# COMP6248-Reproducability-Challenge/selfsupervised-denoising

Measured on AMD Instinct MI355X. Metric: training patches/sec (64x64 gauss25 SSDN), higher is better.
Workload: dtype f16

## Files before the change

include/ssdn_hip.h:

```cpp
#ifndef SSDN_HIP_H
#define SSDN_HIP_H

#include <stdint.h>

#ifdef __cplusplus
extern "C" {
#endif
#if defined(__GNUC__) || defined(__clang__)
#pragma GCC visibility push(default)
#endif

#define SSDN_ABI_VERSION 19
#define SSDN_MAX_TAPS 9

typedef struct ssdn_view {
    void* p;
    int32_t cs;
    int32_t co;
} ssdn_view;

enum ssdn_op_type {
    SSDN_OP_PACK_INPUT = 1,
    SSDN_OP_CONV = 2,
    SSDN_OP_POOL_FWD = 3,
// ... 427 lines not shown
    const float* w_e;
    const float* w_d;
    float* out;
    int32_t B, C, H, W;
    int32_t R;
    int32_t ntaps;
    int32_t dy[SSDN_MAX_TAPS], dx[SSDN_MAX_TAPS];
    const float* add;
} ssdn_input_grad_args;

int ssdn_run_ops(const ssdn_op* ops, int n, void* stream);

int ssdn_stream_order(void* first, void* then);

int ssdn_conv_lds_bytes(const ssdn_conv_args* a);
int ssdn_wgrad_lds_bytes(const ssdn_wgrad_args* a);
int ssdn_wgrad_mega_ok(const ssdn_wgrad_args* a);
int ssdn_wgrad_variant(const ssdn_wgrad_args* a, int32_t* out9);
int ssdn_conv_dma_split(const ssdn_conv_args* a, int32_t* out8);

int ssdn_struct_size(int op_type);
int ssdn_abi_version(void);
const char* ssdn_last_error(void);
int ssdn_device_cus(void);

#define SSDN_PROF_CONV_MT3 0
#define SSDN_PROF_CONV_MT2 1
#define SSDN_PROF_CONV_MT1 2
#define SSDN_PROF_WGRAD 3
#define SSDN_PROF_GEMM 4
#define SSDN_PROF_CDMA_MT3 5
#define SSDN_PROF_CDMA_MT21 6
#define SSDN_PROF_WGRAD_SIDE 7
#define SSDN_PROF_KINDS 8
int ssdn_profile_enable(int kind, int max_launches);
int ssdn_profile_set_stride(int kind, int stride);
int ssdn_profile_read(int kind, double* total_ms, long long* launches, double* flops, double* bytes);

int ssdn_conv_set_mode(int mode);
int ssdn_conv_fuses_pool(const ssdn_conv_args* a);
int ssdn_conv_fuses_upsum(const ssdn_conv_args* a);
int ssdn_conv_fuses_unrot(const ssdn_conv_args* a);
int ssdn_conv_fuses_urot(const ssdn_conv_args* a);
int ssdn_conv_signs(const ssdn_conv_args* a);
int ssdn_conv16_eligible(const ssdn_conv_args* a);
int ssdn_conv_set_conv16(int roles);

int ssdn_chain_len(const ssdn_op* ops, int n);
int ssdn_conv_set_chain(int on);

int ssdn_wgrad_mergeable(const ssdn_wgrad_args* a);

#define SSDN_PLAN_REPACK 0
#define SSDN_PLAN_FORWARD 1
#define SSDN_PLAN_BACKWARD 2
#define SSDN_PLAN_OPTIMISER 3
#define SSDN_PLAN_PHASES 4
typedef struct ssdn_plan ssdn_plan;
int ssdn_plan_load(const void* blob, int64_t nbytes, ssdn_plan** out);
void ssdn_plan_destroy(ssdn_plan* plan);
int64_t ssdn_plan_arena_bytes(const ssdn_plan* plan);
const char* ssdn_plan_meta(const ssdn_plan* plan);
int ssdn_plan_bind(ssdn_plan* plan, void* arena);
int ssdn_plan_tensor(const ssdn_plan* plan, const char* name, void** ptr, int64_t* bytes);
int ssdn_plan_run(ssdn_plan* plan, int phase, void* stream);
int ssdn_plan_set_lr(ssdn_plan* plan, float lr, int step, float gscale);
int ssdn_net_forward(ssdn_plan* plan, void* stream);
int ssdn_train_step(ssdn_plan* plan, float lr, int step, void* stream);

void ssdn_debug_set_trace(void* device_buffer);
void* ssdn_debug_get_trace(void);

int ssdn_probe_mfma(const void* a_frag, const void* b_frag, float* d_out, void* stream);
int ssdn_probe_tr16(const void* lds_image, int image_bytes, const int32_t* lane_addr, void* out, void* stream);

#if defined(__GNUC__) || defined(__clang__)
#pragma GCC visibility pop
#endif
#ifdef __cplusplus
}
#endif
#endif
// ... 1 lines not shown
```

selfsupervised-denoising_amd/csrc/api.hip:

```cpp
#include "common.h"
#include <cstdarg>
#include <cstdio>
#include <cstdlib>

static thread_local char g_err[512] = "";
thread_local hipEvent_t g_ssdn_stop_event = nullptr;
thread_local bool g_ssdn_stop_used = false;
thread_local hipEvent_t g_ssdn_prof_start = nullptr, g_ssdn_prof_stop = nullptr;
thread_local bool g_ssdn_prof_used = false;

int ssdn_set_error(const char* fmt, ...) {
    va_list ap;
    va_start(ap, fmt);
    vsnprintf(g_err, sizeof(g_err), fmt, ap);
    va_end(ap);
    return -1;
}

#include <vector>
struct ProfSlot {
    bool on = false;
    std::vector<hipEvent_t> ev;
    size_t used = 0;
    double flops = 0.0, bytes = 0.0;
// ... 137 lines not shown
int ssdn_conv_lds_bytes(const ssdn_conv_args* a) { return conv_lds_bytes(a); }
int ssdn_wgrad_lds_bytes(const ssdn_wgrad_args* a) { return wgrad_lds_bytes(a); }
int ssdn_wgrad_mergeable(const ssdn_wgrad_args* a) { return a && wgrad_mergeable(a) ? 1 : 0; }
int ssdn_wgrad_mega_ok(const ssdn_wgrad_args* a) { return wgrad_mega_ok(a); }
int ssdn_conv_fuses_pool(const ssdn_conv_args* a) { return a && conv_fuses_pool(a) ? 1 : 0; }
int ssdn_conv_fuses_upsum(const ssdn_conv_args* a) { return a && conv_fuses_upsum(a) ? 1 : 0; }
int ssdn_conv_fuses_unrot(const ssdn_conv_args* a) { return a && conv_fuses_unrot(a) ? 1 : 0; }
int ssdn_conv_fuses_urot(const ssdn_conv_args* a) { return a && conv_fuses_urot(a) ? 1 : 0; }
int ssdn_conv_signs(const ssdn_conv_args* a) { return a && conv_signs(a) ? 1 : 0; }
int ssdn_conv16_eligible(const ssdn_conv_args* a) { return a && conv_use_conv16(a) ? 1 : 0; }

#define SSDN_NEVENTS 256
#define SSDN_NLANES 4
#define SSDN_MAX_DEVICES 16
struct LaneSet {
    hipStream_t side[SSDN_NLANES] = {nullptr, nullptr, nullptr, nullptr};
    hipEvent_t ev[SSDN_NEVENTS];
    int ev_next = 0;
    bool ready = false;
};
static LaneSet g_lanesets[SSDN_MAX_DEVICES];
static LaneSet* lanes_get() {
    int dev = 0;
    if (hipGetDevice(&dev) != hipSuccess || dev < 0 || dev >= SSDN_MAX_DEVICES) { ssdn_set_error("lanes: bad current device"); return nullptr; }
    LaneSet& L = g_lanesets[dev];
    if (L.ready) return &L;
    for (int l = 1; l < SSDN_NLANES; ++l)
        if (hipStreamCreateWithFlags(&L.side[l], hipStreamNonBlocking) != hipSuccess) { ssdn_set_error("lanes: hipStreamCreate failed"); return nullptr; }
    for (int i = 0; i < SSDN_NEVENTS; ++i)
        if (hipEventCreateWithFlags(&L.ev[i], hipEventDisableTiming) != hipSuccess) { ssdn_set_error("lanes: hipEventCreate failed"); return nullptr; }
    L.ready = true;
    return &L;
}
static const unsigned g_lane_deps[SSDN_NLANES] = {0u, 1u << 0, (1u << 0) | (1u << 1) | (1u << 3), 1u << 0};

int ssdn_stream_order(void* first, void* then) {
    LaneSet* LS = lanes_get();
    if (!LS) return -1;
    hipEvent_t e = LS->ev[LS->ev_next++ % SSDN_NEVENTS];
    SSDN_CHECK_HIP(hipEventRecord(e, (hipStream_t)first));
    SSDN_CHECK_HIP(hipStreamWaitEvent((hipStream_t)then, e, 0));
    return 0;
}

int ssdn_run_ops(const ssdn_op* ops, int n, void* stream) {
    hipStream_t lane_s[SSDN_NLANES] = {(hipStream_t)stream, nullptr, nullptr, nullptr};
    g_ssdn_stop_event = nullptr;
    bool dirty[SSDN_NLANES][SSDN_NLANES] = {}, used[SSDN_NLANES] = {true, false, false, false};
    for (int d = 1; d < SSDN_NLANES; ++d) dirty[0][d] = true;
    static const bool one_lane = ssdn_tuning_env("SSDN_ONE_LANE") != nullptr;
    LaneSet* LS = nullptr;
    hipEvent_t cover[SSDN_NLANES] = {nullptr, nullptr, nullptr, nullptr};
    bool covered[SSDN_NLANES] = {false, false, false, false};
    long long cover_at[SSDN_NLANES] = {0, 0, 0, 0};
    auto cover_live = [&](int l) { return covered[l] && (!LS || (long long)LS->ev_next - cover_at[l] < SSDN_NEVENTS - 1); };
    bool has_side = false;
    static const bool no_stop = ssdn_tuning_env("SSDN_NO_STOP_EVENTS") != nullptr;
    for (int i = 0; i < n && !one_lane; ++i) has_side = has_side || ops[i].lane > 0;
    if (has_side && !(LS = lanes_get())) return -1;
    for (int i = 0; i < n; ++i) {
        const void* p = ops[i].args;
        int rc = 0;
        if (!p) return ssdn_set_error("op %d: null args", i);
        int lane = one_lane ? 0 : ops[i].lane;
        if (lane < 0 || lane >= SSDN_NLANES) return ssdn_set_error("op %d: bad lane %d", i, lane);
        if (lane > 0) {
// ... 106 lines not shown
                        if (ok < 0) return -1;
                        if (ok) {
                            arm_last(ia + 1 + mp);
                            rc = launch_tail_fused(items, m, ad, packs, mp, s);
                            i = ia + mp;
                            break;
                        }
                    }
                }
                arm_last(i + m);
                rc = m > 1 ? launch_wreduce_multi(items, m, s) : launch_wreduce((const ssdn_wreduce_args*)p, s);
                i += m - 1;
                break;
            }
            case SSDN_OP_WPACK: {
                const ssdn_wpack_args* items[WPACK_MULTI_MAX];
                int m = 0;
                while (m < WPACK_MULTI_MAX && i + m < n && ops[i + m].type == SSDN_OP_WPACK && ops[i + m].args &&
                       (one_lane ? 0 : ops[i + m].lane) == lane)
                    items[m] = (const ssdn_wpack_args*)ops[i + m].args, ++m;
                rc = m > 1 ? launch_wpack_multi(items, m, s) : launch_wpack((const ssdn_wpack_args*)p, s);
                i += m - 1;
                break;
            }
            case SSDN_OP_GRAD_PACK: {
                const bool next_conv = i + 1 < n && ops[i + 1].type == SSDN_OP_CONV && ops[i + 1].args && (one_lane ? 0 : ops[i + 1].lane) == lane;
                if (next_conv && chain_merging_on() && conv_gradpack_fusable((const ssdn_grad_pack_args*)p, (const ssdn_conv_args*)ops[i + 1].args)) {
                    arm(i + 2);
                    rc = launch_gradpack_dgrad((const ssdn_grad_pack_args*)p, (const ssdn_conv_args*)ops[i + 1].args, s);
                    ++i;
                } else { arm(i + 1); rc = launch_grad_pack((const ssdn_grad_pack_args*)p, s); }
                break;
            }
            case SSDN_OP_HEAD_SSDN: rc = launch_head((const ssdn_head_args*)p, s); break;
            case SSDN_OP_HEAD_FINAL: rc = launch_head_final((const ssdn_head_final_args*)p, s); break;
            case SSDN_OP_SPATIAL_MEAN: rc = launch_spatial_mean((const ssdn_spatial_mean_args*)p, s); break;
            case SSDN_OP_MSE: rc = launch_mse((const ssdn_mse_args*)p, 0, s); break;
            case SSDN_OP_MASK_MSE: rc = launch_mse((const ssdn_mse_args*)p, 1, s); break;
            case SSDN_OP_ADAM: {
                const ssdn_wpack_args* items[ADAM_PACK_MAX];
                int m = 0;
                while (m < ADAM_PACK_MAX && i + 1 + m < n && ops[i + 1 + m].type == SSDN_OP_WPACK && ops[i + 1 + m].args &&
                       (one_lane ? 0 : ops[i + 1 + m].lane) == lane)
                    items[m] = (const ssdn_wpack_args*)ops[i + 1 + m].args, ++m;
                const bool whole_run = !(i + 1 + m < n && ops[i + 1 + m].type == SSDN_OP_WPACK);
                if (m > 0 && whole_run && adam_pack_fusable((const ssdn_adam_args*)p, items, m)) {
                    rc = launch_adam_pack((const ssdn_adam_args*)p, items, m, s);
                    i += m;
                } else rc = launch_adam((const ssdn_adam_args*)p, s);
                break;
            }
            case SSDN_OP_METRICS: rc = launch_metrics((const ssdn_metrics_args*)p, s); break;
            case SSDN_OP_NOISE: rc = launch_noise((const ssdn_noise_args*)p, s); break;
            case SSDN_OP_INPUT_GRAD: arm(i + 1); rc = launch_input_grad((const ssdn_input_grad_args*)p, s); break;
            case SSDN_OP_HEAD_VJP: rc = launch_head_vjp((const ssdn_head_vjp_args*)p, s); break;
            case SSDN_OP_MSE_VJP: rc = launch_mse_vjp((const ssdn_mse_vjp_args*)p, s); break;
            case SSDN_OP_ACCUM: rc = launch_accum((const ssdn_accum_args*)p, s); break;
            case SSDN_OP_HEAD_POSTERIOR: rc = launch_head_posterior((const ssdn_head_posterior_args*)p, s); break;
            case SSDN_OP_SSIM: rc = launch_ssim((const ssdn_ssim_args*)p, s); break;
            case SSDN_OP_CALIBRATION: rc = launch_calibration((const ssdn_calibration_args*)p, s); break;
            case SSDN_OP_IMAGE_IN: rc = launch_image_in((const ssdn_image_in_args*)p, s); break;
            case SSDN_OP_IMAGE_OUT: rc = launch_image_out((const ssdn_image_out_args*)p, s); break;
            case SSDN_OP_NOISE_EST: rc = launch_noise_est((const ssdn_noise_est_args*)p, s); break;
            case SSDN_OP_TILE_IN: rc = launch_tile_in((const ssdn_tile_in_args*)p, s); break;
            case SSDN_OP_TILE_OUT: rc = launch_tile_out((const ssdn_tile_out_args*)p, s); break;
            case SSDN_OP_POOL_PATCH: rc = launch_pool_patch((const ssdn_pool_patch_args*)p, s); break;
            case SSDN_OP_ZERO: {
// ... 75 lines not shown
```

selfsupervised-denoising_amd/csrc/common.h:

```cpp
#pragma once
#include <hip/hip_runtime.h>
#include <hip/hip_ext.h>
#include <stdint.h>
#include "../../include/ssdn_hip.h"
#include <cstdlib>

#if defined(SSDN_TUNING)
static inline const char* ssdn_tuning_env(const char* name) { return std::getenv(name); }
#else
static inline const char* ssdn_tuning_env(const char*) { return nullptr; }
#endif

typedef _Float16 h16;
typedef _Float16 half8 __attribute__((ext_vector_type(8)));
typedef _Float16 half4 __attribute__((ext_vector_type(4)));
typedef _Float16 half2v __attribute__((ext_vector_type(2)));
typedef __bf16 bf16x8 __attribute__((ext_vector_type(8)));
typedef unsigned short u16x8 __attribute__((ext_vector_type(8)));
typedef unsigned short u16x4 __attribute__((ext_vector_type(4)));
typedef float f32x16 __attribute__((ext_vector_type(16)));
typedef float f32x4 __attribute__((ext_vector_type(4)));

#define LRELU_SLOPE 0.1f

// ... 72 lines not shown
static inline int ssdn_current_device_slot() {
    int dev = 0;
    if (hipGetDevice(&dev) != hipSuccess || dev < 0) dev = 0;
    return dev % SSDN_MAX_DEVICES_ATTR;
}

void prof_begin(int kind, hipStream_t s);
void prof_end(int kind, hipStream_t s, double flops, double bytes);

int launch_conv(const ssdn_conv_args* a, hipStream_t s);
int launch_wgrad(const ssdn_wgrad_args* a, hipStream_t s);
bool wgrad_mergeable(const ssdn_wgrad_args* a);
int launch_wgrad_multi(const ssdn_wgrad_args* const* items, int n, hipStream_t s);
#define WGRAD_MEGA_MAX 64
int wgrad_mega_ok(const ssdn_wgrad_args* a);
int launch_wgrad_mega(const ssdn_wgrad_args* const* ops, int n, hipStream_t s);
int launch_pack_input(const ssdn_pack_input_args* a, hipStream_t s);
int launch_pool_fwd(const ssdn_pool_args* a, hipStream_t s);
int launch_pool_bwd(const ssdn_pool_args* a, hipStream_t s);
int launch_upsum_bwd(const ssdn_upsum_args* a, hipStream_t s);
int launch_unrot_fwd(const ssdn_unrot_args* a, hipStream_t s);
int launch_unrot_bwd(const ssdn_unrot_args* a, hipStream_t s);
int launch_wreduce(const ssdn_wreduce_args* a, hipStream_t s);
int launch_wpack(const ssdn_wpack_args* a, hipStream_t s);
#define WPACK_MULTI_MAX 24
int launch_wpack_multi(const ssdn_wpack_args* const* items, int n, hipStream_t s);
#define WREDUCE_MULTI_MAX 32
#define WGRAD_MULTI_MAX 32
int launch_wreduce_multi(const ssdn_wreduce_args* const* items, int n, hipStream_t s);
int launch_grad_pack(const ssdn_grad_pack_args* a, hipStream_t s);
int launch_head(const ssdn_head_args* a, hipStream_t s);
int launch_head_impulse(const ssdn_head_args* a, hipStream_t s);
int launch_head_final(const ssdn_head_final_args* a, hipStream_t s);
int launch_spatial_mean(const ssdn_spatial_mean_args* a, hipStream_t s);
int launch_mse(const ssdn_mse_args* a, int masked, hipStream_t s);
int launch_head_vjp(const ssdn_head_vjp_args* a, hipStream_t s);
int launch_head_vjp_impulse(const ssdn_head_vjp_args* a, hipStream_t s);
int launch_head_posterior(const ssdn_head_posterior_args* a, hipStream_t s);
int launch_ssim(const ssdn_ssim_args* a, hipStream_t s);
int launch_calibration(const ssdn_calibration_args* a, hipStream_t s);
int launch_image_in(const ssdn_image_in_args* a, hipStream_t s);
int launch_image_out(const ssdn_image_out_args* a, hipStream_t s);
int launch_noise_est(const ssdn_noise_est_args* a, hipStream_t s);
int launch_tile_in(const ssdn_tile_in_args* a, hipStream_t s);
int launch_tile_out(const ssdn_tile_out_args* a, hipStream_t s);
int launch_pool_patch(const ssdn_pool_patch_args* a, hipStream_t s);
int launch_mse_vjp(const ssdn_mse_vjp_args* a, hipStream_t s);
int launch_adam(const ssdn_adam_args* a, hipStream_t s);
#define ADAM_PACK_MAX 24
int adam_pack_fusable(const ssdn_adam_args* a, const ssdn_wpack_args* const* items, int n);
int launch_adam_pack(const ssdn_adam_args* a, const ssdn_wpack_args* const* items, int n, hipStream_t s);
int tail_fused_ok(const ssdn_wreduce_args* const* wr, int nw, const ssdn_adam_args* a, const ssdn_wpack_args* const* wp, int np);
int launch_tail_fused(const ssdn_wreduce_args* const* wr, int nw, const ssdn_adam_args* a, const ssdn_wpack_args* const* wp, int np, hipStream_t s);
int launch_metrics(const ssdn_metrics_args* a, hipStream_t s);
int launch_accum(const ssdn_accum_args* a, hipStream_t s);
int launch_noise(const ssdn_noise_args* a, hipStream_t s);
int launch_input_grad(const ssdn_input_grad_args* a, hipStream_t s);
int conv_lds_bytes(const ssdn_conv_args* a);
int conv_validate(const ssdn_conv_args* a);
int chain_len(const ssdn_op* ops, int n, bool any_lane);
int launch_chain(const ssdn_op* ops, int n, bool any_lane, hipStream_t s);
bool chain_merging_on();
bool conv_dma_eligible(const ssdn_conv_args* a, bool any_size);
int conv_dma_lds_bytes(int mt);
bool conv_signs(const ssdn_conv_args* a);
bool gemm_dma_signs(const ssdn_conv_args* a);
// ... 32 lines not shown
```

selfsupervised-denoising_amd/csrc/head.hip:

```cpp
#include "head_math.h"

static constexpr float PME_EPS = 1e-6f;
static __device__ __forceinline__ float diag_pme_weights(float sx, float sn, float& ix, float& in, float& u, float& v) {
    const float e = PME_EPS;
    ix = 1.f / (sx + e);
    in = 1.f / (sn + e);
    const float rD = 1.f / (ix + in + e);
    u = ix * rD;
    v = in * rD;
    return rD;
}

static __device__ __forceinline__ float gauss3_pme_adj(const Sym3& s, Sym3& k) {
    return 1.f / sym3_adj(sym3_add_diag(s, 2 * PME_EPS, 2 * PME_EPS, 2 * PME_EPS), k);
}
template <bool DIAG>
__global__ void k_head(ssdn_head_args a) {
    __shared__ float sh[4];
    const int b = blockIdx.y;
    const long long HW = (long long)a.H * a.W;
    const int C = a.C;
    const int Cout = DIAG ? 2 * C : C + C * (C + 1) / 2;
    const float inv_total = 1.f / ((float)a.B * (float)HW);
    const HeadEst he = head_est(a.mode, a.est_raw, b);
    const float est = he.est, dest_draw = he.dest_draw;
    const float npar = a.noise_param ? a.noise_param[b] : 0.f;
    float loss_acc = 0.f, gest_acc = 0.f, gabs = 0.f;
    const HeadRange r = head_range(HW, a.nchunks);
    const long long p0 = r.p0, p1 = r.p1;
    const float* no = a.net_out + (long long)b * Cout * HW;
    const float* ny = a.noisy + (long long)b * C * HW;
    for (long long p = p0 + threadIdx.x; p < p1; p += HB) {
        if constexpr (DIAG) {
            float mu[3], av[3], sig[3], dsig_dmu[3], dsig_dest[3], sx[3], sn[3], rs[3], q[3];
            float prod = 1.f, quad = 0.f;
#pragma unroll
            for (int c = 0; c < 3; ++c) {
                mu[c] = no[c * HW + p];
                av[c] = no[(3 + c) * HW + p];
                head_sigma(a.style, a.mode, npar, est, mu[c], sig[c], dsig_dmu[c], dsig_dest[c]);
                sx[c] = av[c] * av[c];
                sn[c] = sig[c] * sig[c];
                const float sy = sx[c] + sn[c], d = ny[c * HW + p] - mu[c];
                rs[c] = 1.f / sy;
                q[c] = d * rs[c];
                prod *= sy;
                quad += d * q[c];
            }
            float l = 0.5f * logf(fmaxf(prod, 0.f)) + 0.5f * quad;
            if (a.mode != 0) l -= 0.1f * (sig[0] + sig[1] + sig[2]) * (1.f / 3.f);
            loss_acc += l;
            long long o3 = (long long)b * 3 * HW + p;
            if (a.mu) { a.mu[o3] = mu[0]; a.mu[o3 + HW] = mu[1]; a.mu[o3 + 2 * HW] = mu[2]; }
            if (a.pme) {
#pragma unroll
                for (int c = 0; c < 3; ++c) {
                    float ix, in, u, v;
                    diag_pme_weights(sx[c], sn[c], ix, in, u, v);
                    a.pme[o3 + c * HW] = mu[c] * u + ny[c * HW + p] * v;
                }
            }
            if (a.model_std) a.model_std[(long long)b * HW + p] = cbrtf(fabsf(av[0] * av[1] * av[2]));
            if (a.noise_std && a.style == 1) a.noise_std[(long long)b * HW + p] = cbrtf(sig[0] * sig[1] * sig[2]);
            if (a.want_grad) {
                const float hd = prod > 0.f ? 0.5f : 0.f;
// ... 68 lines not shown
                float t00 = s00 + 2 * e, t11 = s11 + 2 * e, t22 = s22 + 2 * e;
                float k00 = t11 * t22 - s12 * s12, k01 = s02 * s12 - s01 * t22, k02 = s01 * s12 - s02 * t11;
                float k11 = t00 * t22 - s02 * s02, k12 = s01 * s02 - t00 * s12, k22 = t00 * t11 - s01 * s01;
                float rd = 1.f / (t00 * k00 + s01 * k01 + s02 * k02);
                float r0 = (k00 * d0 + k01 * d1 + k02 * d2) * rd;
                float r1 = (k01 * d0 + k11 * d1 + k12 * d2) * rd;
                float r2 = (k02 * d0 + k12 * d1 + k22 * d2) * rd;
                a.pme[o3] = mu[0] + (x00 + e) * r0 + x01 * r1 + x02 * r2;
                a.pme[o3 + HW] = mu[1] + x01 * r0 + (x11 + e) * r1 + x12 * r2;
                a.pme[o3 + 2 * HW] = mu[2] + x02 * r0 + x12 * r1 + (x22 + e) * r2;
            }
            if (a.model_std) a.model_std[(long long)b * HW + p] = cbrtf(fabsf(A[0] * A[3] * A[5]));
            if (a.noise_std && a.style == 1) a.noise_std[(long long)b * HW + p] = cbrtf(sig[0] * sig[1] * sig[2]);
            if (a.want_grad) {
                float hd = det > 0.f ? 0.5f : 0.f;
                const Sym3 G = {hd * i00 - 0.5f * q0 * q0, hd * i01 - 0.5f * q0 * q1, hd * i02 - 0.5f * q0 * q2,
                                hd * i11 - 0.5f * q1 * q1, hd * i12 - 0.5f * q1 * q2, hd * i22 - 0.5f * q2 * q2};
                float reg = a.mode != 0 ? 0.1f / 3.f : 0.f;
                float ds0 = 2.f * sig[0] * G.m00 - reg, ds1 = 2.f * sig[1] * G.m11 - reg, ds2 = 2.f * sig[2] * G.m22 - reg;
                float g[9];
                g[0] = -q0 + ds0 * dsig_dmu[0];
                g[1] = -q1 + ds1 * dsig_dmu[1];
                g[2] = -q2 + ds2 * dsig_dmu[2];
                sym3_dldu(G, A, g + 3);
#pragma unroll
                for (int c = 0; c < 9; ++c) {
                    float v = g[c] * inv_total;
                    a.g_net_out[((long long)b * 9 + c) * HW + p] = v;
                    gabs = fmaxf(gabs, fabsf(v));
                }
                gest_acc += ds0 * dsig_dest[0] + ds1 * dsig_dest[1] + ds2 * dsig_dest[2];
            }
        }
    }
    float ls = block_sum(loss_acc, sh);
    float gs = block_sum(gest_acc, sh);
    if (threadIdx.x == 0) {
        float* pp = a.partial + ((long long)b * a.nchunks + blockIdx.x) * 2;
        pp[0] = ls;
        pp[1] = gs * dest_draw * inv_total;
    }
    if (a.want_grad && a.gmax) atomic_max_abs_block(a.gmax, gabs, sh);
    if (blockIdx.x == 0 && threadIdx.x == 0 && a.noise_std && a.style == 0)
        a.noise_std[b] = head_sigma(0, a.mode, npar, est, 0.f);
}
template <class Args>
static int check_head_args(const char* op, const Args* a, bool need_g) {
    if (a->diag && a->C != 1 && a->C != 3) return ssdn_set_error("%s: diag needs C = 1 or 3", op);
    if (a->C != 1 && a->C != 3) return ssdn_set_error("%s: C must be 1 or 3 (denoiser.py:199)", op);
    if (a->diag != 0 && a->diag != 1) return ssdn_set_error("%s: diag must be 0 or 1", op);
    if (a->B < 1 || a->H < 1 || a->W < 1 || a->nchunks < 1) return ssdn_set_error("%s: bad shape", op);
    if (a->mode < 0 || a->mode > 2 || a->style < 0 || a->style > 2) return ssdn_set_error("%s: bad style / mode", op);
    if (!a->net_out || !a->noisy || !a->partial) return ssdn_set_error("%s: net_out, noisy and partial must be given", op);
    if (need_g && !a->g_net_out) return ssdn_set_error("%s: g_net_out must be given", op);
    if (a->mode == 0 && !a->noise_param) return ssdn_set_error("%s: mode known needs noise_param", op);
    if (a->mode != 0 && !a->est_raw) return ssdn_set_error("%s: modes const / var need est_raw", op);
    return 0;
}
int launch_head(const ssdn_head_args* a, hipStream_t s) {
    if (int rc = check_head_args("head", a, a->want_grad != 0)) return rc;
    if (a->style == 2) return launch_head_impulse(a, s);
    if (a->diag && a->C == 3) hipLaunchKernelGGL(k_head<true>, dim3(a->nchunks, a->B), dim3(HB), 0, s, *a);
    else hipLaunchKernelGGL(k_head<false>, dim3(a->nchunks, a->B), dim3(HB), 0, s, *a);
    return 0;
}

__global__ void k_head_final(ssdn_head_final_args a) {
    int b = blockIdx.x * blockDim.x + threadIdx.x;
    long long HW = (long long)a.H * a.W;
    if (b < a.B) {
        float l = 0.f, g = 0.f;
        for (int c = 0; c < a.nchunks; ++c) {
            l += a.partial[((long long)b * a.nchunks + c) * 2];
            g += a.partial[((long long)b * a.nchunks + c) * 2 + 1];
        }
        if (a.loss) a.loss[b] = l / (float)HW;
        if (a.mode == 2 && a.g_est) a.g_est[b] = g;
    }
    if (a.mode == 1 && a.g_est && b == 0) {
        float g = 0.f;
        for (int bb = 0; bb < a.B; ++bb)
            for (int c = 0; c < a.nchunks; ++c) g += a.partial[((long long)bb * a.nchunks + c) * 2 + 1];
        a.g_est[0] = g;
    }
}
__global__ void k_fill_sigma_grad(ssdn_head_final_args a) {
    long long idx = (long long)blockIdx.x * blockDim.x + threadIdx.x;
    long long HW = (long long)a.H * a.W;
    if (idx >= a.B * HW) return;
    int b = idx / HW;
    float v = a.g_est[b] / (float)HW;
    a.g_sigma_out[idx] = v;
    if ((idx % HW) == 0 && v != 0.f && a.gmax2) atomicMax(a.gmax2, __float_as_uint(fabsf(v)));
}
int launch_head_final(const ssdn_head_final_args* a, hipStream_t s) {
    hipLaunchKernelGGL(k_head_final, dim3((a->B + 63) / 64), dim3(64), 0, s, *a);
    if (a->mode == 2 && a->g_sigma_out) {
        long long n = (long long)a->B * a->H * a->W;
        hipLaunchKernelGGL(k_fill_sigma_grad, dim3((int)((n + 255) / 256)), dim3(256), 0, s, *a);
    }
    return 0;
}

__global__ void k_spatial_mean(ssdn_spatial_mean_args a) {
    __shared__ float sh[4];
    int b = blockIdx.x;
    float acc = 0.f;
    for (int i = threadIdx.x; i < a.HW; i += HB) acc += a.src[(long long)b * a.HW + i];
    float t = block_sum(acc, sh);
    if (threadIdx.x == 0) a.dst[b] = t / (float)a.HW;
}
int launch_spatial_mean(const ssdn_spatial_mean_args* a, hipStream_t s) {
    hipLaunchKernelGGL(k_spatial_mean, dim3(a->B), dim3(HB), 0, s, *a);
    return 0;
}

__global__ void k_mse(ssdn_mse_args a) {
    __shared__ float sh[4];
    int b = blockIdx.x;
    long long n = (long long)a.C * a.H * a.W;
    float acc = 0.f, gabs = 0.f;
    float k = 2.f / ((float)n * (float)a.B);
    for (long long i = threadIdx.x; i < n; i += HB) {
        float d = a.out[b * n + i] - a.ref[b * n + i];
        acc += d * d;
        if (a.g) {
            float g = k * d;
            a.g[b * n + i] = g;
            gabs = fmaxf(gabs, fabsf(g));
        }
    }
    float t = block_sum(acc, sh);
    if (threadIdx.x == 0) a.loss[b] = t / (float)n;
// ... 471 lines not shown
```

selfsupervised-denoising_amd/csrc/head_common.h:

```cpp
#pragma once
#include "common.h"

#define HB 256

static __device__ __forceinline__ float block_sum(float v, float* sh) {
#pragma unroll
    for (int o = 32; o > 0; o >>= 1) v += __shfl_down(v, o, 64);
    int w = threadIdx.x >> 6, l = threadIdx.x & 63;
    __syncthreads();
    if (l == 0) sh[w] = v;
    __syncthreads();
    return sh[0] + sh[1] + sh[2] + sh[3];
}
static __device__ __forceinline__ void atomic_max_abs(uint32_t* gmax, float v) {
    float a = fabsf(v);
#pragma unroll
    for (int o = 32; o > 0; o >>= 1) a = fmaxf(a, __shfl_down(a, o, 64));
    if ((threadIdx.x & 63) == 0 && a > 0.f) atomicMax(gmax, __float_as_uint(a));
}
static __device__ __forceinline__ void atomic_max_abs_block(uint32_t* gmax, float v, float* sh4) {
    float a = fabsf(v);
#pragma unroll
    for (int o = 32; o > 0; o >>= 1) a = fmaxf(a, __shfl_down(a, o, 64));
    __syncthreads();
    if ((threadIdx.x & 63) == 0) sh4[threadIdx.x >> 6] = a;
    __syncthreads();
    if (threadIdx.x == 0) {
        const float m = fmaxf(fmaxf(sh4[0], sh4[1]), fmaxf(sh4[2], sh4[3]));
        if (m > 0.f) atomicMax(gmax, __float_as_uint(m));
    }
}
static __device__ __forceinline__ float softplus_m4(float raw) {
    float x = raw - 4.f;
    return (x > 20.f ? x : log1pf(expf(x))) + 1e-3f;
}
static __device__ __forceinline__ float sigmoid_m4(float raw) {
    float x = raw - 4.f;
    return x > 20.f ? 1.f : 1.f / (1.f + expf(-x));
}
```

selfsupervised-denoising_amd/ssdn/hip/lib.py:

```python
from __future__ import annotations

import ctypes as C
import os

_HERE = os.path.dirname(os.path.abspath(__file__))
LIB_PATH = os.environ.get("SSDN_HIP_LIB") or os.path.join(_HERE, "libssdn_hip.so")
MAX_TAPS = 9

OP = dict(pack_input=1, conv=2, pool_fwd=3, pool_bwd=4, upsum_bwd=5, unrot_fwd=6, unrot_bwd=7, wgrad=8, wreduce=9,
          wpack=10, grad_pack=11, head_ssdn=12, head_final=13, spatial_mean=14, mse=15, mask_mse=16, adam=17,
          metrics=18, zero=19, event_record=20, noise=21, input_grad=22, head_vjp=23,
          mse_vjp=24, accum=25, head_posterior=26, ssim=27, calibration=28, image_in=29, image_out=30, noise_est=31,
          tile_in=32, tile_out=33, pool_patch=34)

i32, f32, vp = C.c_int32, C.c_float, C.c_void_p


class View(C.Structure):
    _fields_ = [("p", vp), ("cs", i32), ("co", i32)]


class OpRec(C.Structure):
    _fields_ = [("type", i32), ("lane", i32), ("args", vp)]

# ... 168 lines not shown
                ("k0", i32), ("B", i32), ("dst", vp)]


class TileOutArgs(C.Structure):
    _fields_ = [("store", vp), ("w", i32), ("h", i32), ("C", i32), ("T", i32), ("O", i32), ("Kx", i32), ("Ky", i32), ("mode", i32),
                ("dst", vp), ("dst_bytes", C.c_int64)]


class PoolPatchArgs(C.Structure):
    _fields_ = [("pool", vp), ("offsets", vp), ("sizes", vp), ("params", vp), ("index", vp), ("noisy32", vp), ("ref32", vp), ("coords", vp),
                ("param_out", vp), ("origin_out", vp), ("N", i32), ("B", i32), ("C", i32), ("P", i32), ("augment", i32),
                ("n2v_box", i32), ("n2v_radius", i32), ("seed", C.c_uint64), ("offset", C.c_uint64)]


def tile_count(n: int, T: int, O: int) -> int:
    return 1 if n <= T else -(-(n - O) // (T - O))


ARG_TYPES = dict(pack_input=PackInputArgs, conv=ConvArgs, pool_fwd=PoolArgs, pool_bwd=PoolArgs, upsum_bwd=UpsumArgs,
                 unrot_fwd=UnrotArgs, unrot_bwd=UnrotArgs, wgrad=WgradArgs, wreduce=WreduceArgs, wpack=WpackArgs,
                 grad_pack=GradPackArgs, head_ssdn=HeadArgs, head_final=HeadFinalArgs, spatial_mean=SpatialMeanArgs,
                 mse=MseArgs, mask_mse=MseArgs, adam=AdamArgs, metrics=MetricsArgs, zero=ZeroArgs, event_record=EventArgs, noise=NoiseArgs,
                 input_grad=InputGradArgs, head_vjp=HeadVjpArgs, mse_vjp=MseVjpArgs, accum=AccumArgs,
                 head_posterior=HeadPosteriorArgs, ssim=SsimArgs, calibration=CalibrationArgs, image_in=ImageInArgs, image_out=ImageOutArgs,
                 noise_est=NoiseEstArgs, tile_in=TileInArgs, tile_out=TileOutArgs, pool_patch=PoolPatchArgs)

ABI_VERSION = 19

SYMBOLS = ["ssdn_run_ops", "ssdn_stream_order", "ssdn_conv_lds_bytes", "ssdn_wgrad_lds_bytes", "ssdn_abi_version", "ssdn_last_error",
           "ssdn_device_cus", "ssdn_probe_mfma", "ssdn_probe_tr16", "ssdn_struct_size", "ssdn_profile_enable",
           "ssdn_profile_read", "ssdn_profile_set_stride", "ssdn_debug_set_trace", "ssdn_debug_get_trace", "ssdn_conv_set_mode",
           "ssdn_wgrad_mergeable", "ssdn_conv_fuses_pool", "ssdn_conv_fuses_upsum", "ssdn_conv_fuses_unrot", "ssdn_conv_fuses_urot", "ssdn_conv_signs", "ssdn_chain_len",
           "ssdn_conv_set_chain", "ssdn_wgrad_mega_ok", "ssdn_wgrad_variant", "ssdn_conv_dma_split", "ssdn_conv16_eligible", "ssdn_conv_set_conv16",
           "ssdn_plan_load", "ssdn_plan_destroy", "ssdn_plan_arena_bytes", "ssdn_plan_meta", "ssdn_plan_bind", "ssdn_plan_tensor", "ssdn_plan_run",
           "ssdn_plan_set_lr", "ssdn_net_forward", "ssdn_train_step"]
PLAN_PHASES = dict(repack=0, forward=1, backward=2, optimiser=3)
PROF = dict(conv_mt3=0, conv_mt2=1, conv_mt1=2, wgrad=3, gemm=4, cdma_mt3=5, cdma_mt21=6, wgrad_side=7)

CONV_SIGN_FIELDS = ("unrot_smask", "urot_smask", "sign_out", "mask_sign", "upsum_mask_sign")


def conv_args(a: dict, view, ptr) -> ConvArgs:
    s = ConvArgs()
    s.src0, s.src1 = view(a["src0"]), view(a["src1"])
    s.c0, s.c1, s.up0, s.N, s.H, s.W, s.ntaps = a["c0"], a["c1"], a["up0"], a["N"], a["H"], a["W"], len(a["taps"])
    for t, (dy, dx) in enumerate(a["taps"]):
        s.dy[t], s.dx[t] = dy, dx
    s.w, s.wc = ptr("w", a["layer"]), ptr("wc", a["layer"])
    s.M, s.Mpad, s.Ktot, s.act = a["M"], a["Mpad"], a["Ktot"], a["act"]
    s.bias = ptr("bias", a["layer"]) if a["bias"] else None
    s.mask, s.add, s.dst = view(a["mask"]), view(a["add"]), view(a["dst"])
    s.dst32 = ptr("dst32", a["dst32"]) if a["dst32"] is not None else None
    s.ltw, s.lth, s.ltn, s.kc, s.bf16, s.kreal = a["ltw"], a["lth"], a["ltn"], a["kc"], a["bf16"], a.get("kreal", 0)
    s.pool, s.pool_shifted = view(a.get("pool")), a.get("pool_shifted", 0)
    s.upsum, s.upsum_mask, s.upsum_c = view(a.get("upsum")), view(a.get("upsum_mask")), a.get("upsum_c", 0)
    s.unrot, s.unrot_mask, s.urot = view(a.get("unrot")), view(a.get("unrot_mask")), view(a.get("urot"))
    for k in CONV_SIGN_FIELDS:
        setattr(s, k, ptr(k, a[k]) if a.get(k) is not None else None)
    return s


def pointer_fields(st, base: int = 0):
    out = []
    for name, ty in st._fields_:
        off = base + getattr(st, name).offset
        if ty is vp:
            out.append(off)
        elif isinstance(ty, type) and issubclass(ty, C.Structure):
            out += pointer_fields(ty, off)
    return out
# ... 27 lines not shown
    lib.ssdn_last_error.restype = C.c_char_p
    lib.ssdn_device_cus.restype = C.c_int
    lib.ssdn_probe_mfma.argtypes = [vp, vp, vp, vp]
    lib.ssdn_probe_mfma.restype = C.c_int
    lib.ssdn_probe_tr16.argtypes = [vp, C.c_int, vp, vp, vp]
    lib.ssdn_probe_tr16.restype = C.c_int
    lib.ssdn_profile_enable.argtypes = [C.c_int, C.c_int]
    lib.ssdn_profile_enable.restype = C.c_int
    lib.ssdn_profile_set_stride.argtypes = [C.c_int, C.c_int]
    lib.ssdn_profile_set_stride.restype = C.c_int
    lib.ssdn_profile_read.argtypes = [C.c_int, C.POINTER(C.c_double), C.POINTER(C.c_longlong), C.POINTER(C.c_double), C.POINTER(C.c_double)]
    lib.ssdn_profile_read.restype = C.c_int
    lib.ssdn_conv_set_mode.argtypes = [C.c_int]
    lib.ssdn_conv_set_mode.restype = C.c_int
    lib.ssdn_conv_set_chain.argtypes = [C.c_int]
    lib.ssdn_conv_set_chain.restype = C.c_int
    lib.ssdn_chain_len.argtypes = [C.c_void_p, C.c_int]
    lib.ssdn_chain_len.restype = C.c_int
    lib.ssdn_conv_fuses_unrot.argtypes = [C.c_void_p]
    lib.ssdn_conv_fuses_unrot.restype = C.c_int
    lib.ssdn_conv_fuses_urot.argtypes = [C.c_void_p]
    lib.ssdn_conv_fuses_urot.restype = C.c_int
    lib.ssdn_conv_signs.argtypes = [C.c_void_p]
    lib.ssdn_conv_signs.restype = C.c_int
    lib.ssdn_conv_fuses_upsum.argtypes = [C.c_void_p]
    lib.ssdn_conv_fuses_upsum.restype = C.c_int
    lib.ssdn_conv_fuses_pool.argtypes = [C.c_void_p]
    lib.ssdn_conv_fuses_pool.restype = C.c_int
    if hasattr(lib, "ssdn_conv16_eligible"):
        lib.ssdn_conv16_eligible.argtypes = [C.c_void_p]
        lib.ssdn_conv16_eligible.restype = C.c_int
        lib.ssdn_conv_set_conv16.argtypes = [C.c_int]
        lib.ssdn_conv_set_conv16.restype = C.c_int
    lib.ssdn_wgrad_mergeable.argtypes = [C.c_void_p]
    lib.ssdn_wgrad_mergeable.restype = C.c_int
    lib.ssdn_wgrad_mega_ok.argtypes = [C.c_void_p]
    lib.ssdn_wgrad_mega_ok.restype = C.c_int
    lib.ssdn_wgrad_variant.argtypes = [C.c_void_p, C.POINTER(C.c_int32)]
    lib.ssdn_wgrad_variant.restype = C.c_int
    if hasattr(lib, "ssdn_conv_dma_split"):
        lib.ssdn_conv_dma_split.argtypes = [C.c_void_p, C.POINTER(C.c_int32)]
        lib.ssdn_conv_dma_split.restype = C.c_int
    lib.ssdn_struct_size.argtypes = [C.c_int]
    lib.ssdn_struct_size.restype = C.c_int
    lib.ssdn_plan_load.argtypes = [C.c_void_p, C.c_int64, C.POINTER(C.c_void_p)]
    lib.ssdn_plan_load.restype = C.c_int
    lib.ssdn_plan_destroy.argtypes = [C.c_void_p]
    lib.ssdn_plan_destroy.restype = None
    lib.ssdn_plan_arena_bytes.argtypes = [C.c_void_p]
    lib.ssdn_plan_arena_bytes.restype = C.c_int64
    lib.ssdn_plan_meta.argtypes = [C.c_void_p]
    lib.ssdn_plan_meta.restype = C.c_char_p
    lib.ssdn_plan_bind.argtypes = [C.c_void_p, C.c_void_p]
    lib.ssdn_plan_bind.restype = C.c_int
    lib.ssdn_plan_tensor.argtypes = [C.c_void_p, C.c_char_p, C.POINTER(C.c_void_p), C.POINTER(C.c_int64)]
    lib.ssdn_plan_tensor.restype = C.c_int
    lib.ssdn_plan_run.argtypes = [C.c_void_p, C.c_int, C.c_void_p]
    lib.ssdn_plan_run.restype = C.c_int
    lib.ssdn_plan_set_lr.argtypes = [C.c_void_p, C.c_float, C.c_int, C.c_float]
    lib.ssdn_plan_set_lr.restype = C.c_int
    lib.ssdn_net_forward.argtypes = [C.c_void_p, C.c_void_p]
    lib.ssdn_net_forward.restype = C.c_int
    lib.ssdn_train_step.argtypes = [C.c_void_p, C.c_float, C.c_int, C.c_void_p]
    lib.ssdn_train_step.restype = C.c_int
    if lib.ssdn_abi_version() != ABI_VERSION:
        raise SsdnHipError("libssdn_hip.so ABI version mismatch")
    if os.environ.get("SSDN_CHAIN_MODE"):
        lib.ssdn_conv_set_chain(int(os.environ["SSDN_CHAIN_MODE"]))
    if os.environ.get("SSDN_CONV16_ROLES") and hasattr(lib, "ssdn_conv_set_conv16"):
        lib.ssdn_conv_set_conv16(int(os.environ["SSDN_CONV16_ROLES"]))
    _lib = lib
    return lib


def check(rc: int):
    if rc != 0:
        raise SsdnHipError(load().ssdn_last_error().decode())
```

Baseline: 21020.

## Fuse head final reduction into head kernel and widen head blocks

Adds a last-block-done pattern so the head kernel performs the final per-batch loss/gradient reduction itself, using an atomic counter ring and agent-scope atomics, which removes a separate k_head_final launch. It also adds a 'wide' head variant that launches up to 2-4x more threads per block, staging per-pixel partials in LDS and reducing them, to raise parallelism within each chunk. Both add atomic and synchronization overhead, and the wide path uses more LDS and is only taken for some shapes. Profiling slots for head kernels are added as well.

After: 21020, median of 3. No clear change (-0.0%).

```diff
diff --git a/include/ssdn_hip.h b/include/ssdn_hip.h
--- a/include/ssdn_hip.h
+++ b/include/ssdn_hip.h
@@ -483,7 +483,9 @@
 #define SSDN_PROF_CDMA_MT3 5
 #define SSDN_PROF_CDMA_MT21 6
 #define SSDN_PROF_WGRAD_SIDE 7
-#define SSDN_PROF_KINDS 8
+#define SSDN_PROF_HEAD 8
+#define SSDN_PROF_HEAD_FINAL 9
+#define SSDN_PROF_KINDS 10
 int ssdn_profile_enable(int kind, int max_launches);
 int ssdn_profile_set_stride(int kind, int stride);
 int ssdn_profile_read(int kind, double* total_ms, long long* launches, double* flops, double* bytes);
@@ -499,6 +501,8 @@
 
 int ssdn_chain_len(const ssdn_op* ops, int n);
 int ssdn_conv_set_chain(int on);
+
+int ssdn_head_set_wide(int on);
 
 int ssdn_wgrad_mergeable(const ssdn_wgrad_args* a);
 
diff --git a/selfsupervised-denoising_amd/csrc/api.hip b/selfsupervised-denoising_amd/csrc/api.hip
--- a/selfsupervised-denoising_amd/csrc/api.hip
+++ b/selfsupervised-denoising_amd/csrc/api.hip
@@ -193,6 +193,28 @@
     L.ready = true;
     return &L;
 }
+#define SSDN_NCOUNTERS 256
+struct CounterRing {
+    unsigned* dev = nullptr;
+    unsigned next = 0;
+};
+static CounterRing g_counters[SSDN_MAX_DEVICES];
+static unsigned* counter_draw() {
+    int dev = 0;
+    if (hipGetDevice(&dev) != hipSuccess || dev < 0 || dev >= SSDN_MAX_DEVICES) { ssdn_set_error("counters: bad current device"); return nullptr; }
+    CounterRing& R = g_counters[dev];
+    if (!R.dev) {
+        unsigned* p = nullptr;
+        if (hipMalloc((void**)&p, sizeof(unsigned) * SSDN_NCOUNTERS) != hipSuccess) { ssdn_set_error("counters: hipMalloc failed"); return nullptr; }
+        if (hipMemset(p, 0, sizeof(unsigned) * SSDN_NCOUNTERS) != hipSuccess || hipDeviceSynchronize() != hipSuccess) {
+            (void)hipFree(p);
+            ssdn_set_error("counters: hipMemset failed");
+            return nullptr;
+        }
+        R.dev = p;
+    }
+    return R.dev + R.next++ % SSDN_NCOUNTERS;
+}
 static const unsigned g_lane_deps[SSDN_NLANES] = {0u, 1u << 0, (1u << 0) | (1u << 1) | (1u << 3), 1u << 0};
 
 int ssdn_stream_order(void* first, void* then) {
@@ -365,7 +387,16 @@
                 } else { arm(i + 1); rc = launch_grad_pack((const ssdn_grad_pack_args*)p, s); }
                 break;
             }
-            case SSDN_OP_HEAD_SSDN: rc = launch_head((const ssdn_head_args*)p, s); break;
+            case SSDN_OP_HEAD_SSDN: {
+                const bool next_final = i + 1 < n && ops[i + 1].type == SSDN_OP_HEAD_FINAL && ops[i + 1].args && (one_lane ? 0 : ops[i + 1].lane) == lane;
+                if (next_final && chain_merging_on() && head_final_fusable((const ssdn_head_args*)p, (const ssdn_head_final_args*)ops[i + 1].args)) {
+                    unsigned* counter = counter_draw();
+                    if (!counter) return -1;
+                    rc = launch_head_with_final((const ssdn_head_args*)p, (const ssdn_head_final_args*)ops[i + 1].args, counter, s);
+                    if (!rc) ++i;
+                } else rc = launch_head((const ssdn_head_args*)p, s);
+                break;
+            }
             case SSDN_OP_HEAD_FINAL: rc = launch_head_final((const ssdn_head_final_args*)p, s); break;
             case SSDN_OP_SPATIAL_MEAN: rc = launch_spatial_mean((const ssdn_spatial_mean_args*)p, s); break;
             case SSDN_OP_MSE: rc = launch_mse((const ssdn_mse_args*)p, 0, s); break;
diff --git a/selfsupervised-denoising_amd/csrc/common.h b/selfsupervised-denoising_amd/csrc/common.h
--- a/selfsupervised-denoising_amd/csrc/common.h
+++ b/selfsupervised-denoising_amd/csrc/common.h
@@ -128,6 +128,8 @@
 int launch_head(const ssdn_head_args* a, hipStream_t s);
 int launch_head_impulse(const ssdn_head_args* a, hipStream_t s);
 int launch_head_final(const ssdn_head_final_args* a, hipStream_t s);
+bool head_final_fusable(const ssdn_head_args* a, const ssdn_head_final_args* f);
+int launch_head_with_final(const ssdn_head_args* a, const ssdn_head_final_args* f, unsigned* counter, hipStream_t s);
 int launch_spatial_mean(const ssdn_spatial_mean_args* a, hipStream_t s);
 int launch_mse(const ssdn_mse_args* a, int masked, hipStream_t s);
 int launch_head_vjp(const ssdn_head_vjp_args* a, hipStream_t s);
diff --git a/selfsupervised-denoising_amd/csrc/head.hip b/selfsupervised-denoising_amd/csrc/head.hip
--- a/selfsupervised-denoising_amd/csrc/head.hip
+++ b/selfsupervised-denoising_amd/csrc/head.hip
@@ -14,9 +14,38 @@
 static __device__ __forceinline__ float gauss3_pme_adj(const Sym3& s, Sym3& k) {
     return 1.f / sym3_adj(sym3_add_diag(s, 2 * PME_EPS, 2 * PME_EPS, 2 * PME_EPS), k);
 }
-template <bool DIAG>
-__global__ void k_head(ssdn_head_args a) {
+template <bool COHERENT>
+static __device__ __forceinline__ float head_partial_load(const float* p) {
+    if constexpr (COHERENT) return __hip_atomic_load(p, __ATOMIC_RELAXED, __HIP_MEMORY_SCOPE_AGENT);
+    else return *p;
+}
+template <bool COHERENT>
+static __device__ __forceinline__ void head_final_sums(const ssdn_head_final_args& a, int b0, int bstep) {
+    const long long HW = (long long)a.H * a.W;
+    for (int b = b0; b < a.B; b += bstep) {
+        float l = 0.f, g = 0.f;
+        for (int c = 0; c < a.nchunks; ++c) {
+            l += head_partial_load<COHERENT>(a.partial + ((long long)b * a.nchunks + c) * 2);
+            g += head_partial_load<COHERENT>(a.partial + ((long long)b * a.nchunks + c) * 2 + 1);
+        }
+        if (a.loss) a.loss[b] = l / (float)HW;
+        if (a.mode == 2 && a.g_est) a.g_est[b] = g;
+    }
+    if (a.mode == 1 && a.g_est && b0 == 0) {
+        float g = 0.f;
+        for (int bb = 0; bb < a.B; ++bb)
+            for (int c = 0; c < a.nchunks; ++c) g += head_partial_load<COHERENT>(a.partial + ((long long)bb * a.nchunks + c) * 2 + 1);
+        a.g_est[0] = g;
+    }
+}
+struct HeadFin {
+    ssdn_head_final_args fa;
+    unsigned* counter;
+};
+template <bool DIAG, bool WIDE, bool FIN>
+__global__ void k_head(ssdn_head_args a, HeadFin f) {
     __shared__ float sh[4];
+    extern __shared__ float shw[];
     const int b = blockIdx.y;
     const long long HW = (long long)a.H * a.W;
     const int C = a.C;
@@ -30,7 +59,8 @@
     const long long p0 = r.p0, p1 = r.p1;
     const float* no = a.net_out + (long long)b * Cout * HW;
     const float* ny = a.noisy + (long long)b * C * HW;
-    for (long long p = p0 + threadIdx.x; p < p1; p += HB) {
+    for (long long p = p0 + threadIdx.x; p < p1; p += WIDE ? (int)blockDim.x : HB) {
+        if constexpr (WIDE) loss_acc = gest_acc = 0.f;
         if constexpr (DIAG) {
             float mu[3], av[3], sig[3], dsig_dmu[3], dsig_dest[3], sx[3], sn[3], rs[3], q[3];
             float prod = 1.f, quad = 0.f;
@@ -165,17 +195,50 @@
                 gest_acc += ds0 * dsig_dest[0] + ds1 * dsig_dest[1] + ds2 * dsig_dest[2];
             }
         }
-    }
-    float ls = block_sum(loss_acc, sh);
-    float gs = block_sum(gest_acc, sh);
+        if constexpr (WIDE) reinterpret_cast<float2*>(shw + HEAD_WIDE_MAX_WAVES)[(int)(p - p0)] = make_float2(loss_acc, gest_acc);
+    }
+    if constexpr (WIDE) {
+        __syncthreads();
+        loss_acc = gest_acc = 0.f;
+        if (threadIdx.x < HB)
+            for (long long p = p0 + threadIdx.x; p < p1; p += HB) {
+                const float2 v = reinterpret_cast<const float2*>(shw + HEAD_WIDE_MAX_WAVES)[(int)(p - p0)];
+                loss_acc += v.x;
+                gest_acc += v.y;
+            }
+    }
+    float ls = WIDE ? block_sum_first256(loss_acc, sh) : block_sum(loss_acc, sh);
+    float gs = WIDE ? block_sum_first256(gest_acc, sh) : block_sum(gest_acc, sh);
     if (threadIdx.x == 0) {
         float* pp = a.partial + ((long long)b * a.nchunks + blockIdx.x) * 2;
-        pp[0] = ls;
-        pp[1] = gs * dest_draw * inv_total;
-    }
-    if (a.want_grad && a.gmax) atomic_max_abs_block(a.gmax, gabs, sh);
+        if constexpr (FIN) {
+            __hip_atomic_store(pp, ls, __ATOMIC_RELAXED, __HIP_MEMORY_SCOPE_AGENT);
+            __hip_atomic_store(pp + 1, gs * dest_draw * inv_total, __ATOMIC_RELAXED, __HIP_MEMORY_SCOPE_AGENT);
+        } else {
+            pp[0] = ls;
+            pp[1] = gs * dest_draw * inv_total;
+        }
+    }
+    if (a.want_grad && a.gmax) {
+        if constexpr (WIDE) atomic_max_abs_wide(a.gmax, gabs, shw);
+        else atomic_max_abs_block(a.gmax, gabs, sh);
+    }
     if (blockIdx.x == 0 && threadIdx.x == 0 && a.noise_std && a.style == 0)
         a.noise_std[b] = head_sigma(0, a.mode, npar, est, 0.f);
+    if constexpr (FIN) {
+        __shared__ int last;
+        if (threadIdx.x == 0) {
+            asm volatile("s_waitcnt vmcnt(0)" ::: "memory");
+            const unsigned t = __hip_atomic_fetch_add(f.counter, 1u, __ATOMIC_RELAXED, __HIP_MEMORY_SCOPE_AGENT);
+            last = t == gridDim.x * gridDim.y - 1;
+        }
+        __syncthreads();
+        if (last) {
+            __builtin_amdgcn_fence(__ATOMIC_ACQUIRE, "agent");
+            head_final_sums<true>(f.fa, threadIdx.x, blockDim.x);
+            if (threadIdx.x == 0) __hip_atomic_store(f.counter, 0u, __ATOMIC_RELAXED, __HIP_MEMORY_SCOPE_AGENT);
+        }
+    }
 }
 template <class Args>
 static int check_head_args(const char* op, const Args* a, bool need_g) {
@@ -190,32 +253,42 @@
     if (a->mode != 0 && !a->est_raw) return ssdn_set_error("%s: modes const / var need est_raw", op);
     return 0;
 }
+static int g_head_wide = 1;
+extern "C" int ssdn_head_set_wide(int on) {
+    if (on < 0 || on > 2) return ssdn_set_error("ssdn_head_set_wide: 0, 1 or 2");
+    g_head_wide = on;
+    return 0;
+}
+template <bool DIAG>
+static void head_dispatch(const ssdn_head_args* a, const HeadFin& f, bool fin, hipStream_t s) {
+    const long long HW = (long long)a->H * a->W, per = (HW + a->nchunks - 1) / a->nchunks, R = (per + HB - 1) / HB;
+    const dim3 grid(a->nchunks, a->B);
+    const bool fused_gest = a->C == 1 && a->want_grad && a->mode != 0;
+    if (g_head_wide && !fused_gest && R >= 2 && R <= HEAD_WIDE_MAX_ROUNDS) {
+        const int cap = g_head_wide == 2 ? 4 : 2, Rp = R < cap ? (int)R : cap;
+        const size_t lds = sizeof(float) * (HEAD_WIDE_MAX_WAVES + 2 * (size_t)R * HB);
+        if (fin) hipLaunchKernelGGL((k_head<DIAG, true, true>), grid, dim3(HB * Rp), lds, s, *a, f);
+        else hipLaunchKernelGGL((k_head<DIAG, true, false>), grid, dim3(HB * Rp), lds, s, *a, f);
+    } else if (fin) hipLaunchKernelGGL((k_head<DIAG, false, true>), grid, dim3(HB), 0, s, *a, f);
+    else hipLaunchKernelGGL((k_head<DIAG, false, false>), grid, dim3(HB), 0, s, *a, f);
+}
+static int launch_head_impl(const ssdn_head_args* a, const HeadFin& f, bool fin, hipStream_t s) {
+    if (int rc = check_head_args("head", a, a->want_grad != 0)) return rc;
+    prof_begin(SSDN_PROF_HEAD, s);
+    int rc = 0;
+    if (a->style == 2) rc = launch_head_impulse(a, s);
+    else if (a->diag && a->C == 3) head_dispatch<true>(a, f, fin, s);
+    else head_dispatch<false>(a, f, fin, s);
+    prof_end(SSDN_PROF_HEAD, s, 0.0, 0.0);
+    return rc;
+}
 int launch_head(const ssdn_head_args* a, hipStream_t s) {
-    if (int rc = check_head_args("head", a, a->want_grad != 0)) return rc;
-    if (a->style == 2) return launch_head_impulse(a, s);
-    if (a->diag && a->C == 3) hipLaunchKernelGGL(k_head<true>, dim3(a->nchunks, a->B), dim3(HB), 0, s, *a);
-    else hipLaunchKernelGGL(k_head<false>, dim3(a->nchunks, a->B), dim3(HB), 0, s, *a);
-    return 0;
+    const HeadFin none = {};
+    return launch_head_impl(a, none, false, s);
 }
 
 __global__ void k_head_final(ssdn_head_final_args a) {
-    int b = blockIdx.x * blockDim.x + threadIdx.x;
-    long long HW = (long long)a.H * a.W;
-    if (b < a.B) {
-        float l = 0.f, g = 0.f;
-        for (int c = 0; c < a.nchunks; ++c) {
-            l += a.partial[((long long)b * a.nchunks + c) * 2];
-            g += a.partial[((long long)b * a.nchunks + c) * 2 + 1];
-        }
-        if (a.loss) a.loss[b] = l / (float)HW;
-        if (a.mode == 2 && a.g_est) a.g_est[b] = g;
-    }
-    if (a.mode == 1 && a.g_est && b == 0) {
-        float g = 0.f;
-        for (int bb = 0; bb < a.B; ++bb)
-            for (int c = 0; c < a.nchunks; ++c) g += a.partial[((long long)bb * a.nchunks + c) * 2 + 1];
-        a.g_est[0] = g;
-    }
+    head_final_sums<false>(a, blockIdx.x * blockDim.x + threadIdx.x, gridDim.x * blockDim.x);
 }
 __global__ void k_fill_sigma_grad(ssdn_head_final_args a) {
     long long idx = (long long)blockIdx.x * blockDim.x + threadIdx.x;
@@ -226,12 +299,27 @@
     a.g_sigma_out[idx] = v;
     if ((idx % HW) == 0 && v != 0.f && a.gmax2) atomicMax(a.gmax2, __float_as_uint(fabsf(v)));
 }
-int launch_head_final(const ssdn_head_final_args* a, hipStream_t s) {
-    hipLaunchKernelGGL(k_head_final, dim3((a->B + 63) / 64), dim3(64), 0, s, *a);
+static void launch_fill_sigma_grad(const ssdn_head_final_args* a, hipStream_t s) {
     if (a->mode == 2 && a->g_sigma_out) {
         long long n = (long long)a->B * a->H * a->W;
         hipLaunchKernelGGL(k_fill_sigma_grad, dim3((int)((n + 255) / 256)), dim3(256), 0, s, *a);
     }
+}
+int launch_head_final(const ssdn_head_final_args* a, hipStream_t s) {
+    prof_begin(SSDN_PROF_HEAD_FINAL, s);
+    hipLaunchKernelGGL(k_head_final, dim3((a->B + 63) / 64), dim3(64), 0, s, *a);
+    prof_end(SSDN_PROF_HEAD_FINAL, s, 0.0, 0.0);
+    launch_fill_sigma_grad(a, s);
+    return 0;
+}
+bool head_final_fusable(const ssdn_head_args* a, const ssdn_head_final_args* f) {
+    return a->style != 2 && f->partial == a->partial && f->B == a->B && f->nchunks == a->nchunks && f->H == a->H && f->W == a->W &&
+           f->mode == a->mode;
+}
+int launch_head_with_final(const ssdn_head_args* a, const ssdn_head_final_args* fa, unsigned* counter, hipStream_t s) {
+    const HeadFin f = {*fa, counter};
+    if (int rc = launch_head_impl(a, f, true, s)) return rc;
+    launch_fill_sigma_grad(fa, s);
     return 0;
 }
 
diff --git a/selfsupervised-denoising_amd/csrc/head_common.h b/selfsupervised-denoising_amd/csrc/head_common.h
--- a/selfsupervised-denoising_amd/csrc/head_common.h
+++ b/selfsupervised-denoising_amd/csrc/head_common.h
@@ -30,6 +30,30 @@
         if (m > 0.f) atomicMax(gmax, __float_as_uint(m));
     }
 }
+#define HEAD_WIDE_MAX_ROUNDS 16
+#define HEAD_WIDE_MAX_WAVES 16
+static __device__ __forceinline__ float block_sum_first256(float v, float* sh) {
+#pragma unroll
+    for (int o = 32; o > 0; o >>= 1) v += __shfl_down(v, o, 64);
+    int w = threadIdx.x >> 6, l = threadIdx.x & 63;
+    __syncthreads();
+    if (l == 0 && w < 4) sh[w] = v;
+    __syncthreads();
+    return sh[0] + sh[1] + sh[2] + sh[3];
+}
+static __device__ __forceinline__ void atomic_max_abs_wide(uint32_t* gmax, float v, float* shw) {
+    float a = fabsf(v);
+#pragma unroll
+    for (int o = 32; o > 0; o >>= 1) a = fmaxf(a, __shfl_down(a, o, 64));
+    __syncthreads();
+    if ((threadIdx.x & 63) == 0) shw[threadIdx.x >> 6] = a;
+    __syncthreads();
+    if (threadIdx.x == 0) {
+        float m = 0.f;
+        for (int w = 0; w < (int)(blockDim.x >> 6); ++w) m = fmaxf(m, shw[w]);
+        if (m > 0.f) atomicMax(gmax, __float_as_uint(m));
+    }
+}
 static __device__ __forceinline__ float softplus_m4(float raw) {
     float x = raw - 4.f;
     return (x > 20.f ? x : log1pf(expf(x))) + 1e-3f;
diff --git a/selfsupervised-denoising_amd/ssdn/hip/lib.py b/selfsupervised-denoising_amd/ssdn/hip/lib.py
--- a/selfsupervised-denoising_amd/ssdn/hip/lib.py
+++ b/selfsupervised-denoising_amd/ssdn/hip/lib.py
@@ -224,10 +224,13 @@
            "ssdn_profile_read", "ssdn_profile_set_stride", "ssdn_debug_set_trace", "ssdn_debug_get_trace", "ssdn_conv_set_mode",
            "ssdn_wgrad_mergeable", "ssdn_conv_fuses_pool", "ssdn_conv_fuses_upsum", "ssdn_conv_fuses_unrot", "ssdn_conv_fuses_urot", "ssdn_conv_signs", "ssdn_chain_len",
            "ssdn_conv_set_chain", "ssdn_wgrad_mega_ok", "ssdn_wgrad_variant", "ssdn_conv_dma_split", "ssdn_conv16_eligible", "ssdn_conv_set_conv16",
+           "ssdn_head_set_wide",
            "ssdn_plan_load", "ssdn_plan_destroy", "ssdn_plan_arena_bytes", "ssdn_plan_meta", "ssdn_plan_bind", "ssdn_plan_tensor", "ssdn_plan_run",
            "ssdn_plan_set_lr", "ssdn_net_forward", "ssdn_train_step"]
 PLAN_PHASES = dict(repack=0, forward=1, backward=2, optimiser=3)
 PROF = dict(conv_mt3=0, conv_mt2=1, conv_mt1=2, wgrad=3, gemm=4, cdma_mt3=5, cdma_mt21=6, wgrad_side=7)
+
+PROF_HEAD = dict(head=8, head_final=9)
 
 CONV_SIGN_FIELDS = ("unrot_smask", "urot_smask", "sign_out", "mask_sign", "upsum_mask_sign")
 
@@ -321,6 +324,9 @@
         lib.ssdn_conv16_eligible.restype = C.c_int
         lib.ssdn_conv_set_conv16.argtypes = [C.c_int]
         lib.ssdn_conv_set_conv16.restype = C.c_int
+    if hasattr(lib, "ssdn_head_set_wide"):
+        lib.ssdn_head_set_wide.argtypes = [C.c_int]
+        lib.ssdn_head_set_wide.restype = C.c_int
     lib.ssdn_wgrad_mergeable.argtypes = [C.c_void_p]
     lib.ssdn_wgrad_mergeable.restype = C.c_int
     lib.ssdn_wgrad_mega_ok.argtypes = [C.c_void_p]
@@ -358,6 +364,8 @@
         lib.ssdn_conv_set_chain(int(os.environ["SSDN_CHAIN_MODE"]))
     if os.environ.get("SSDN_CONV16_ROLES") and hasattr(lib, "ssdn_conv_set_conv16"):
         lib.ssdn_conv_set_conv16(int(os.environ["SSDN_CONV16_ROLES"]))
+    if os.environ.get("SSDN_HEAD_WIDE") and hasattr(lib, "ssdn_head_set_wide"):
+        lib.ssdn_head_set_wide(int(os.environ["SSDN_HEAD_WIDE"]))
     _lib = lib
     return lib
 
```
